# AllenNeuralDynamics/aind-smartspim-destripe

Measured on AMD Instinct MI355X. Metric: 2048x2048 uint16 slices/s destriped, higher is better.
Workload: dtype f32

## Files before the change

### aind_smartspim_destripe_amd/csrc/dsx.hip

```cpp
#include <hip/hip_runtime.h>
#include <dlfcn.h>
#include <math.h>
#include <rccl/rccl.h>
#include <stdio.h>
#include <stdlib.h>
#include <string.h>

#include <string>
#include <vector>

#include "../../include/dsx.h"
#include "dsx_kernels.h"
#include "dsx_retile.h"
#include "dsx_pyramid.h"
#include "dsx_wavelet.h"
#include "dsx_plan.h"
#include "dsx_io.h"
#include "dsx_streaks.h"
#include "dsx_zenc_kernels.h"
#include "dsx_zdec_kernels.h"

namespace {

thread_local std::string g_init_error;
// ... 3 lines not shown
                                     "k_rowfilter",       "k_inv_march(pyramid)", "k_inv_march(final)"};

struct ProfRec {
  int cls;
  hipEvent_t e0, e1;
};

}

struct DsxTuning {
  int row_wpb = 0;
  int march_waves = 256 * 16;
  bool no_quant = false;
  int seg_min_rows = 4;
  bool no_fuse = false;
  bool no_fuse_inv = false;
  bool no_pair = false;
  int hist_rows = 0;
  int fwd_wpb = 8, inv_wpb = 8;
  bool no_row_multi = false;
  int row_multi_alone = 48;
  int helper = -1;
  bool no_pipeline = false;
#ifdef DSX_DIAG
  int skip_hist = 0, skip_row = 0, skip_from = 1000;
#endif
};

struct dsx_ctx {
  int device = 0;
  DsxTuning tune;
  hipStream_t stream_ = nullptr;
  std::string err;
  bool planned = false;
  dsx::Plan plan;
  dsx::HostCfg cfg[2];
  double high_int = 2700.0;
  int max_batch = 0;
  float fg_cutoff = 383.12503f;
  float* d_ws = nullptr;
  char* d_ctl = nullptr;
  size_t ctl_zero_bytes = 0;
  dsx::PlaneStats* d_stats = nullptr;
  unsigned* d_minmax = nullptr;
  unsigned* d_hist = nullptr;
  float* d_thr = nullptr;
  float* d_otsu = nullptr;
  int* d_cfg = nullptr;
  double* d_means = nullptr;
  dsx::C32* d_consts = nullptr;
  size_t consts_bytes = 0;
  float* d_flat = nullptr;
  float* d_dark = nullptr;
  bool own_shading = false;
  int dark_h = 0, dark_w = 0;
  void* d_stage_in = nullptr;
  void* d_stage_out = nullptr;
  size_t stage_in_bytes = 0, stage_out_bytes = 0;
  int last_n = 0;
  int stop_after = 0;
  hipEvent_t t0 = nullptr, t1 = nullptr;
  bool profiling = false;
  std::vector<ProfRec> prof;
  size_t workspace_bytes = 0;
  int wl_len = 0;
  int wl_bank_len = 0;
  bool wl_set = false;
  float wl[4][dsx::kMaxTaps] = {};
  float wl_bank[4][dsx::kMaxTaps] = {};
  unsigned* h_sticky = nullptr;
  uint8_t* zenc_slots = nullptr;
  uint32_t* zenc_sizes = nullptr;
  size_t zenc_blocks = 0;
  uint8_t* zenc_lits = nullptr;
  size_t zenc_lit_blocks = 0;
  uint8_t* zdec_scratch = nullptr;
  size_t zdec_bytes = 0;
  unsigned* d_sticky = nullptr;
  bool stack_mode = false;
  bool no_fuse_rf = false;
  bool fuse_rf_wide = false;
  int ablate = 0;
// ... 65 lines not shown
}

int env_int(const char* name, int fallback) {
  const char* v = getenv(name);
  return (v && *v) ? atoi(v) : fallback;
}

void read_tuning(DsxTuning& t) {
  t.row_wpb = env_int("DSX_ROW_WPB", 0);
  if (t.row_wpb != 0) t.row_wpb = std::max(4, std::min(t.row_wpb, (int)dsx::kRowMaxWaves));
  t.march_waves = std::max(64, env_int("DSX_MARCH_WAVES", 256 * 16));
  t.no_quant = env_int("DSX_NO_QUANT", 0) != 0;
  t.seg_min_rows = std::max(2, env_int("DSX_SEG_MIN_ROWS", 4));
  t.no_fuse = env_int("DSX_NO_FUSE", 0) != 0;
  t.no_fuse_inv = env_int("DSX_NO_FUSE_INV", 0) != 0;
  t.no_pair = env_int("DSX_NO_PAIR", 0) != 0;
  t.hist_rows = std::max(0, env_int("DSX_HIST_ROWS", 0));
  t.fwd_wpb = env_int("DSX_FWD_WPB", 8) == 4 ? 4 : 8;
  t.inv_wpb = env_int("DSX_INV_WPB", 8) == 4 ? 4 : 8;
  t.no_row_multi = env_int("DSX_NO_ROW_MULTI", 0) != 0;
  t.row_multi_alone = std::max(0, env_int("DSX_ROW_MULTI_ALONE", 48));
  t.helper = getenv("DSX_HELPER") ? (env_int("DSX_HELPER", 0) != 0 ? 1 : 0) : -1;
  t.no_pipeline = env_int("DSX_NO_PIPELINE", 0) != 0;
#ifdef DSX_DIAG
  t.skip_hist = env_int("DSX_SKIP_HIST", 0);
  t.skip_row = env_int("DSX_SKIP_ROW", 0);
  t.skip_from = env_int("DSX_SKIP_COARSE", 1000);
#endif
}

int fail(dsx_ctx* c, int code, const std::string& msg) {
  if (c) c->err = msg;
  else g_init_error = msg;
  return code;
}

hipStream_t use_main(dsx_ctx* c) {
  for (int i = 1; i < c->joins_pending; ++i) (void)hipStreamWaitEvent(c->stream_, c->ev_join[i], 0);
  c->joins_pending = 0;
  ++c->main_ops;
  return c->stream_;
}

#define DSX_HIP(call)                                                                    \
  do {                                                                                   \
    hipError_t e_ = (call);                                                              \
// ... 3 lines not shown

void drop_graphs(dsx_ctx* c) {
  for (auto& g : c->graphs)
    if (g.exec) (void)hipGraphExecDestroy(g.exec);
  c->graphs.clear();
}

void free_plan_buffers(dsx_ctx* c) {
  drop_graphs(c);
  auto fr = [](void* p) { if (p) (void)hipFree(p); };
  fr(c->d_ws); c->d_ws = nullptr;
  fr(c->d_ctl); c->d_ctl = nullptr;
  fr(c->d_thr); c->d_thr = nullptr;
  fr(c->d_otsu); c->d_otsu = nullptr;
  fr(c->d_cfg); c->d_cfg = nullptr;
  fr(c->d_means); c->d_means = nullptr;
  fr(c->d_consts); c->d_consts = nullptr;
  if (c->own_shading) { fr(c->d_flat); fr(c->d_dark); }
  c->d_flat = c->d_dark = nullptr;
  c->own_shading = false;
  fr(c->d_stage_in); c->d_stage_in = nullptr; c->stage_in_bytes = 0;
  fr(c->d_stage_out); c->d_stage_out = nullptr; c->stage_out_bytes = 0;
  c->planned = false;
}

struct LaunchScope {
  dsx_ctx* c;
  bool on;
  ProfRec r;
  LaunchScope(dsx_ctx* c_, int cls) : c(c_), on(c_->profiling) {
    if (on) {
      r.cls = cls;
      (void)hipEventCreate(&r.e0);
      (void)hipEventCreate(&r.e1);
      (void)hipEventRecord(r.e0, c->stream_);
    }
  }
  ~LaunchScope() {
    if (on) {
      (void)hipEventRecord(r.e1, c->stream_);
      c->prof.push_back(r);
    }
  }
};

int rowfilter_waves_per_block(int M) {
// ... 23 lines not shown
  const int wpb = force_wpb ? force_wpb : ((CPL > 18 || a_in.M >= 1024) ? 4 : rowfilter_waves_per_block(a_in.M));
  const size_t smem = (size_t)a_in.M * (wpb + 1) * sizeof(float2);
  const dsx::RowArgs& a = a_in;
  const dim3 grid((npairs + wpb - 1) / wpb, nb);
  hipLaunchKernelGGL((dsx::k_rowfilter<CPL, GF, NT, HALO, PLAN>), grid, dim3(64 * wpb), smem, s, a);
  return hipGetLastError();
}

hipError_t launch_rowfilter_wide(const dsx::RowArgs& a, int npairs, int nb, hipStream_t s) {
  static bool attr_set[64] = {};
  int dev = 0;
  (void)hipGetDevice(&dev);
  if (!attr_set[dev & 63]) {
    hipError_t e = hipFuncSetAttribute((const void*)dsx::k_rowfilter_wide, hipFuncAttributeMaxDynamicSharedMemorySize,
                                       (int)(dsx::kWideMaxLen * sizeof(float2)));
    if (e != hipSuccess) return e;
    attr_set[dev & 63] = true;
  }
  if (a.M > dsx::kWideMaxLen || a.w >= 65536) return hipErrorInvalidValue;
  hipLaunchKernelGGL(dsx::k_rowfilter_wide, dim3(npairs, nb), dim3(dsx::kWideThreads), (size_t)a.M * sizeof(float2), s, a);
  return hipGetLastError();
}

hipError_t dispatch_rowfilter(const dsx::RowArgs& a, int npairs, int nb, hipStream_t s) {
  const int cpl = (a.M + 63) / 64;
  if (cpl > 36) return launch_rowfilter_wide(a, npairs, nb, s);
  const int gf = a.w >> 8, nt = (a.w - (gf << 8) + 63) >> 6;
  auto plan_is = [&](int m, int r0, int r1, int r2) {
    return a.M == m && a.npass == 3 && a.radix[0] == r0 && a.radix[1] == r1 && a.radix[2] == r2;
  };
  if (cpl <= 2) return launch_rowfilter<2>(a, npairs, nb, s);
  if (cpl <= 4) return launch_rowfilter<4>(a, npairs, nb, s);
  if (cpl <= 6) return launch_rowfilter<6>(a, npairs, nb, s);
  if (cpl <= 10) return launch_rowfilter<10>(a, npairs, nb, s);
  if (cpl <= 18) {
    if (gf == 4 && nt == 1 && a.K == 0) {
      if (plan_is(1026, 19, 9, 6))
        return launch_rowfilter<18, 4, 1, 0, 1>(a, npairs, nb, s);
      return launch_rowfilter<18, 4, 1, 0>(a, npairs, nb, s);
    }
    if (gf == 2 && nt == 1 && a.K > 0) {
      if (plan_is(1071, 17, 9, 7))
        return launch_rowfilter<18, 2, 1, 1, 2>(a, npairs, nb, s);
      return launch_rowfilter<18, 2, 1, 1>(a, npairs, nb, s);
    }
    if (gf == 1 && nt == 4 && a.K > 0) {
      if (plan_is(1024, 16, 8, 8)) return launch_rowfilter<18, 1, 4, 1, 5>(a, npairs, nb, s);
      if (plan_is(960, 15, 8, 8)) return launch_rowfilter<18, 1, 4, 1, 6>(a, npairs, nb, s);
    }
// ... 28 lines not shown
  if (!attr_set[dev & 63]) {
    hipError_t e = hipFuncSetAttribute((const void*)kern, hipFuncAttributeMaxDynamicSharedMemorySize, 160 * 1024);
    if (e != hipSuccess) return e;
    attr_set[dev & 63] = true;
  }
  const size_t smem = (size_t)a.r.M * (dsx::kRfWaves + 1) * sizeof(float2);
  const int np = (a.f.hout + 1) / 2;
  int nblk = (np + dsx::kRfRows - 1) / dsx::kRfRows;
#if DSX_RF_XCD
  nblk = (nblk + 7) / 8 * 8;
#endif
  const dim3 grid(nblk, nb);
  hipLaunchKernelGGL(kern, grid, dim3(64 * dsx::kRfWaves), smem, s, a);
  return hipGetLastError();
}

hipError_t launch_rowfinal(int plan, const dsx::RowFinalArgs& a, int nb, hipStream_t s) {
  if (plan == 1) return launch_rowfinal_t<18, 4, 1, 0, 1>(a, nb, s);
  if (plan == 3) return launch_rowfinal_t<36, 3, 4, 1, 3>(a, nb, s);
  if (plan == 4) return launch_rowfinal_t<36, 3, 3, 1, 4>(a, nb, s);
  return hipErrorInvalidValue;
}

hipError_t launch_rowfilter_multi(const dsx::RowMultiArgs& a_in, const int* npairs, int nb, hipStream_t s) {
  static bool attr_set[64] = {};
  int dev = 0;
  (void)hipGetDevice(&dev);
  if (!attr_set[dev & 63]) {
    hipError_t e = hipFuncSetAttribute((const void*)dsx::k_rowfilter_multi<6>, hipFuncAttributeMaxDynamicSharedMemorySize, 160 * 1024);
    if (e != hipSuccess) return e;
    attr_set[dev & 63] = true;
  }
  const int wpb = dsx::kRowMaxWaves;
  dsx::RowMultiArgs a = a_in;
  int blocks = 0, max_m = 1;
  for (int i = 0; i < a.nlev; ++i) {
    blocks += (npairs[i] + wpb - 1) / wpb;
    a.blk_end[i] = blocks;
    max_m = std::max(max_m, a.lv[i].M);
  }
  const size_t smem = (size_t)max_m * (wpb + 1) * sizeof(float2);
  hipLaunchKernelGGL(dsx::k_rowfilter_multi<6>, dim3(blocks, nb), dim3(64 * wpb), smem, s, a);
  return hipGetLastError();
}

void march_segments(int nb, int nstrips, int rows, int* nseg, int* rows_per_seg, int wpb = 0, int halo_rows = 0,
                    bool coarse = false) {
  const int target_waves = tune().march_waves;
  const bool no_quant = tune().no_quant;
  int want = (target_waves + nb * nstrips - 1) / (nb * nstrips);
  const int seg_min_coarse = tune().seg_min_rows;
  const int seg_min_rows = coarse ? seg_min_coarse : 24;
  const int max_seg = std::max(1, rows / seg_min_rows);
  want = std::max(1, std::min(want, max_seg));
  if (wpb > 0 && !no_quant) {
    static int cus = 0;
    if (cus == 0) {
      int dev = 0;
      hipDeviceProp_t prop;
      if (hipGetDevice(&dev) == hipSuccess && hipGetDeviceProperties(&prop, dev) == hipSuccess) cus = prop.multiProcessorCount;
      if (cus <= 0) cus = 256;
    }
    const long long slots = (long long)cus * (16 / wpb);
    double best = 1e300;
    int best_n = want;
// ... 188 lines not shown
    a.sticky = ctx->d_sticky;
    a.shared = ctx->stack_mode ? 1 : 0;
    LaunchScope ls(ctx, KC_OTSU);
    hipLaunchKernelGGL(dsx::k_otsu, dim3(L, nb), dim3(64), 0, s, a);
    DSX_HIP(hipGetLastError());
    if (d_cfg_used)
      DSX_HIP(hipMemcpyAsync(d_cfg_used, v.cfg, sizeof(int32_t) * nb, hipMemcpyDeviceToDevice, s));
  } else if (d_cfg_used) {
    DSX_HIP(hipMemsetAsync(d_cfg_used, 0, sizeof(int32_t) * nb, s));
  }
  if (ctx->stop_after == 1) return DSX_OK;

  const bool split_inv = split && fuse21;
  if (split_inv) {
    DSX_HIP(hipEventRecord(v.ev[2], s));
    DSX_HIP(hipStreamWaitEvent(v.helper, v.ev[2], 0));
  }
  dsx::RowArgs row1;
  memset(&row1, 0, sizeof(row1));
  const bool no_multi = ctx->tune.no_row_multi;
  dsx::RowMultiArgs multi;
  memset(&multi, 0, sizeof(multi));
  int multi_pairs[dsx::kRowMultiMax] = {};
  for (int l = 0; l < L && l < skip_from; ++l) {
    hipStream_t rs = (split_inv && l < 2) ? v.helper : s;
    if ((skip_row >> l) & 1) continue;
    const dsx::LevelPlan& lp = p.lv[l];
    dsx::RowArgs a;
    memset(&a, 0, sizeof(a));
    a.ws = v.ws;
    a.ws_plane_stride = p.plane_floats;
    a.da_off = lp.da_off;
    a.h = lp.h; a.w = lp.w; a.ld = lp.ld;
    a.thr = v.thr;
    a.cfg = v.cfg;
    a.lvl = l; a.L = L;
    a.lvl_active[0] = p.cfg_levels[0];
    a.lvl_active[1] = p.cfg_levels[1];
    a.M = lp.M; a.K = lp.K;
    a.npass = lp.npass;
    for (int i = 0; i < lp.npass; ++i) a.radix[i] = lp.radix[i];
    a.tw = (const float2*)(ctx->d_consts + lp.tw_off);
    a.g[0] = (const float2*)(ctx->d_consts + lp.g_off[0]);
    a.g[1] = (const float2*)(ctx->d_consts + lp.g_off[1]);
    a.kcut[0] = lp.kcut[0];
    a.kcut[1] = lp.kcut[1];
    a.inv_M = 1.0f / (float)lp.M;
    a.ablate = ctx->ablate;
    if (fuse_rf && l == 0) {
      row1 = a;
      continue;
    }
    const int npairs = (lp.h + 1) / 2;
    const int multi_alone = ctx->tune.row_multi_alone;
    if (!no_multi && (!v.alone || nb <= multi_alone) && rs == s && a.M <= 6 * 64 && multi.nlev < dsx::kRowMultiMax) {
      multi_pairs[multi.nlev] = npairs;
      multi.lv[multi.nlev++] = a;
      continue;
    }
    LaunchScope ls(ctx, KC_ROW);
    DSX_HIP(dispatch_rowfilter(a, npairs, nb, rs));
  }
  if (multi.nlev == 1) {
    LaunchScope ls(ctx, KC_ROW);
    DSX_HIP(dispatch_rowfilter(multi.lv[0], multi_pairs[0], nb, s));
  } else if (multi.nlev > 1) {
    LaunchScope ls(ctx, KC_ROW);
    DSX_HIP(launch_rowfilter_multi(multi, multi_pairs, nb, s));
  }
  if (split_inv) DSX_HIP(hipEventRecord(v.ev[3], v.helper));
  if (ctx->stop_after == 2) return DSX_OK;

  for (int l = L - 1; l >= (L > 0 ? 0 : -1); --l) {
    if (fuse21 && l == 1) continue;
    if (l >= skip_from) continue;
    if (generic) {
      dsx::GenInvArgs g;
      memset(&g, 0, sizeof(g));
      const dsx::LevelPlan& lp = p.lv[l];
      g.ws = v.ws;
      g.ws_plane_stride = p.plane_floats;
      g.c_off = lp.aa_off; g.d_off = lp.da_off;
      g.hc = lp.h; g.wc = lp.w; g.ldc = lp.lda; g.ldd = lp.ld;
      g.has_c = (l < L - 1) ? 1 : 0;
      g.has_pyr = 1;
      g.F = ctx->wl_len;
      memcpy(g.lo, ctx->wl[2], sizeof(float) * ctx->wl_len);
      memcpy(g.hi, ctx->wl[3], sizeof(float) * ctx->wl_len);
      const bool last_g = (l == 0);
      if (!last_g) {
        const dsx::LevelPlan& lo = p.lv[l - 1];
// ... 1432 lines not shown
  DSX_HIP(hipStreamSynchronize(use_main(ctx)));
  if (int rc = check_sticky(ctx)) return rc;
  double m[2];
  int c = 0;
  DSX_HIP(hipMemcpy(m, ctx->d_means + 2 * plane, sizeof(m), hipMemcpyDeviceToHost));
  DSX_HIP(hipMemcpy(&c, ctx->d_cfg + plane, sizeof(int), hipMemcpyDeviceToHost));
  if (fore_mean) *fore_mean = m[0];
  if (back_mean) *back_mean = m[1];
  if (cfg_used) *cfg_used = c;
  return DSX_OK;
}
int dsx_get_thresholds(dsx_ctx* ctx, int plane, int level, float* otsu, float* threshold) {
  if (!ctx) return DSX_EINVAL;
  if (!ctx->planned) return fail(ctx, DSX_ENOPLAN, "dsx_plan has not been called");
  if (plane < 0 || plane >= ctx->last_n || level < 0 || level >= ctx->plan.L)
    return fail(ctx, DSX_EINVAL, "plane / level index out of range");
  DSX_HIP(hipSetDevice(ctx->device));
  DSX_HIP(hipStreamSynchronize(use_main(ctx)));
  const size_t i = (size_t)plane * ctx->plan.L + level;
  if (otsu) DSX_HIP(hipMemcpy(otsu, ctx->d_otsu + i, sizeof(float), hipMemcpyDeviceToHost));
  if (threshold) DSX_HIP(hipMemcpy(threshold, ctx->d_thr + i, sizeof(float), hipMemcpyDeviceToHost));
  return DSX_OK;
}
int dsx_get_level(dsx_ctx* ctx, int plane, int level, int stage, float* out) {
  if (!ctx || !out) return DSX_EINVAL;
  if (!ctx->planned) return fail(ctx, DSX_ENOPLAN, "dsx_plan has not been called");
  if (plane < 0 || plane >= ctx->last_n || level < 0 || level >= ctx->plan.L)
    return fail(ctx, DSX_EINVAL, "plane / level index out of range");
  DSX_HIP(hipSetDevice(ctx->device));
  DSX_HIP(hipStreamSynchronize(use_main(ctx)));
  const dsx::LevelPlan& lp = ctx->plan.lv[level];
  const long long off = (stage == DSX_STAGE_APPROX) ? lp.aa_off : lp.da_off;
  const int pitch = (stage == DSX_STAGE_APPROX) ? lp.lda : lp.ld;
  const float* src = ctx->d_ws + (size_t)plane * ctx->plan.plane_floats + off;
  DSX_HIP(hipMemcpy2D(out, sizeof(float) * lp.w, src, sizeof(float) * pitch, sizeof(float) * lp.w, lp.h,
                      hipMemcpyDeviceToHost));
  return DSX_OK;
}

int dsx_plan_streaks(dsx_ctx* ctx, int height, int width, int max_batch, const dsx_streaks_cfg* cfg) {
  if (!ctx) return DSX_EINVAL;
  if (!cfg) return fail(ctx, DSX_EINVAL, "config is NULL");
  if (height < 1 || width < 1) return fail(ctx, DSX_EINVAL, "plane must be at least 1 x 1");
  if (max_batch < 1) return fail(ctx, DSX_EINVAL, "max_batch must be >= 1");
  if (!(cfg->sigma_fg > 0.f) || !(cfg->sigma_bg > 0.f)) return fail(ctx, DSX_EINVAL, "sigma must be positive");
  if (!(cfg->crossover > 0.f)) return fail(ctx, DSX_EINVAL, "crossover must be positive");
// ... 81 lines not shown
```

### aind_smartspim_destripe_amd/csrc/dsx_kernels.h

```cpp
#ifndef DSX_KERNELS_H
#define DSX_KERNELS_H

#include <type_traits>
#include <hip/hip_runtime.h>
#include <stdint.h>

#include "dsx_fft_core.h"

#ifndef DSX_NT
#define DSX_NT 1
#endif
#ifndef DSX_MEDIAN_BALLOT
#define DSX_MEDIAN_BALLOT 1
#endif
#ifndef DSX_FWD_STEADY
#define DSX_FWD_STEADY 1
#endif
#ifndef DSX_RF_XCD
#define DSX_RF_XCD 0
#endif
#ifndef DSX_INV_MINW
#define DSX_INV_MINW 1
#endif
#ifndef DSX_FWD_PRUNE
#define DSX_FWD_PRUNE 1
#endif
#ifndef DSX_SWZ
#define DSX_SWZ 1
#endif
#ifndef DSX_FWD_MINW
// ... 1053 lines not shown
    const double t = fmin(otsu >= 0 ? sqrt(otsu) : 0.0, (double)a.max_thr[cfg]);
    a.otsu[pl] = (float)otsu;
    a.thr[pl] = (float)t;
  }
}

struct RowArgs {
  float* ws;
  long long ws_plane_stride;
  long long da_off;
  int h, w, ld;
  const float* thr;
  const int* cfg;
  int lvl, L;
  int lvl_active[2];
  int M, K;
  int npass;
  int radix[kMaxPasses];
  const float2* tw;
  const float2* g[2];
  int kcut[2];
  float inv_M;
  int ablate;
};

__device__ __forceinline__ unsigned f32_key(float v) {
  const unsigned b = as_u32(v);
  return (b & 0x80000000u) ? ~b : (b | 0x80000000u);
}
__device__ __forceinline__ float key_f32(unsigned k) {
  return as_f32((k & 0x80000000u) ? (k & 0x7FFFFFFFu) : ~k);
}

template <int R, int CPL, int JK = (R - 1) / 2, int KO = (R - 1) / 2, class IX = dsx_idx_plain>
__device__ __forceinline__ void fft_pass(float2* buf, const float2* tw, int M, int s, float inv_s,
                                         int lane) {
  constexpr int MAXB = (CPL + R - 1) / R;
  const int nb = M / R;
  const bool unit_tw = (s * R == M);
  dsx_c32 v[MAXB][R];
#pragma unroll
  for (int i = 0; i < MAXB; ++i) {
    const int b = lane + kWave * i;
    if (b < nb) dsx_bfly_load<R, JK, IX>((const dsx_c32*)buf, b, nb, v[i]);
  }
  wave_sync();
// ... 143 lines not shown
    const int jk = (kcut + 53) / 54;
    if (jk <= 2) run_first_pruned<CPL, 2>(buf, tw, lane);
    else if (jk <= 4) run_first_pruned<CPL, 4>(buf, tw, lane);
    else run<CPL>(buf, tw, lane);
  }
};
template <>
struct StaticFft<2> {
  static constexpr int M = 1071;
  static constexpr bool kSwz = false;
  static constexpr int kRadix[3] = {17, 9, 7};
  template <int CPL>
  static __device__ __forceinline__ void run(float2* buf, const float2* tw, int lane) {
    fft_static_passes<CPL, 1071, 1, 17, 9, 7>(buf, tw, lane);
  }
  template <int CPL>
  static __device__ __forceinline__ void run_forward(float2* buf, const float2* tw, int lane, int) { run<CPL>(buf, tw, lane); }
  template <int CPL>
  static __device__ __forceinline__ void run_inverse(float2* buf, const float2* tw, int lane, int) {
    run<CPL>(buf, tw, lane);
  }
};

#define DSX_STATIC_FFT(ID, LEN, R0, R1, R2, SWZ)                                                   \
  template <>                                                                                      \
  struct StaticFft<ID> {                                                                           \
    static constexpr int M = LEN;                                                                  \
    static constexpr bool kSwz = SWZ;                                                              \
    template <int CPL>                                                                             \
    static __device__ __forceinline__ void run(float2* buf, const float2* tw, int lane) {          \
      if constexpr (SWZ) fft_static_passes_swz<CPL, LEN, 1, R0, R1, R2>(buf, tw, lane);            \
      else fft_static_passes<CPL, LEN, 1, R0, R1, R2>(buf, tw, lane);                              \
    }                                                                                              \
    template <int CPL>                                                                             \
    static __device__ __forceinline__ void run_forward(float2* buf, const float2* tw, int lane, int) { \
      run<CPL>(buf, tw, lane);                                                                     \
    }                                                                                              \
    template <int CPL>                                                                             \
    static __device__ __forceinline__ void run_inverse(float2* buf, const float2* tw, int lane, int) { \
      run<CPL>(buf, tw, lane);                                                                     \
    }                                                                                              \
  };
DSX_STATIC_FFT(3, 2048, 16, 16, 8, DSX_SWZ != 0)
DSX_STATIC_FFT(4, 1815, 15, 11, 11, false)
DSX_STATIC_FFT(5, 1024, 16, 8, 8, DSX_SWZ != 0)
DSX_STATIC_FFT(6, 960, 15, 8, 8, false)
#undef DSX_STATIC_FFT

typedef short dsx_s16x2 __attribute__((ext_vector_type(2)));

__device__ __forceinline__ dsx_s16x2 as_s16x2(unsigned u) {
  union { unsigned u; dsx_s16x2 v; } c;
  c.u = u;
  return c.v;
}
__device__ __forceinline__ unsigned as_u32(dsx_s16x2 v) {
  union { unsigned u; dsx_s16x2 v; } c;
  c.v = v;
  return c.u;
}

template <int CPL>
struct RowSlots {
  static constexpr int GV = CPL / 4;
  static constexpr int E = 4 * GV + 4;
};
template <int E>
struct SlotMask { typedef unsigned long long type; };
template <> struct SlotMask<4> { typedef unsigned type; };
template <> struct SlotMask<8> { typedef unsigned type; };
// ... 371 lines not shown
  const int tid = threadIdx.x, lane = tid & 63, wave = tid >> 6;
  const int M = (PLAN_ > 0) ? StaticFft<PLAN_>::M : a.M;
  rf_pair_body<CPL, GF_, NT_, HALO_, PLAN_, false>(a, dsx_smem, dsx_smem + (long long)M * (1 + wave), tid, blockDim.x, lane,
                                                   blockIdx.x * (blockDim.x >> 6) + wave, blockIdx.y);
}

constexpr int kRowMultiMax = 8;
struct RowMultiArgs {
  int nlev;
  int blk_end[kRowMultiMax];
  RowArgs lv[kRowMultiMax];
};

template <int CPL>
__global__ __launch_bounds__(64 * kRowMaxWaves, row_waves_per_simd<CPL>()) void k_rowfilter_multi(RowMultiArgs args) {
  extern __shared__ __attribute__((aligned(16))) float2 dsx_smem[];
  const int tid = threadIdx.x, lane = tid & 63, wave = tid >> 6;
  int ent = 0;
  while (ent + 1 < args.nlev && (int)blockIdx.x >= args.blk_end[ent]) ++ent;
  const RowArgs& a = args.lv[ent];
  const int bx = (int)blockIdx.x - (ent > 0 ? args.blk_end[ent - 1] : 0);
  rf_pair_body<CPL, -1, -1, -1, 0, false>(a, dsx_smem, dsx_smem + (long long)a.M * (1 + wave), tid, blockDim.x, lane,
                                          bx * (blockDim.x >> 6) + wave, blockIdx.y);
}

constexpr int kWideThreads = 512;
constexpr int kWideCpl = 36;
constexpr int kWideMaxLen = kWideThreads * kWideCpl;

__device__ __forceinline__ unsigned wide_block_sum(unsigned v, unsigned* s_red, int& turn) {
  v = __reduce_add_sync(~0ull, v);
  unsigned* slot = s_red + ((turn & 1) ? (kWideThreads / 64) : 0);
  if ((threadIdx.x & 63) == 0) slot[threadIdx.x >> 6] = v;
  __syncthreads();
  unsigned t = 0;
#pragma unroll
  for (int w = 0; w < kWideThreads / 64; ++w) t += slot[w];
  ++turn;
  return t;
}
__device__ __forceinline__ unsigned wide_block_min(unsigned v, unsigned* s_red, int& turn) {
  v = __reduce_min_sync(~0ull, v);
  unsigned* slot = s_red + ((turn & 1) ? (kWideThreads / 64) : 0);
  if ((threadIdx.x & 63) == 0) slot[threadIdx.x >> 6] = v;
  __syncthreads();
  unsigned t = ~0u;
// ... 889 lines not shown
```

### aind_smartspim_destripe_amd/csrc/dsx_plan.h

```cpp
#ifndef DSX_PLAN_H
#define DSX_PLAN_H

#include <math.h>
#include <stdint.h>
#include <stdlib.h>

#include <algorithm>
#include <string>
#include <vector>

namespace dsx {

constexpr int kPlanMaxLevels = 16;
constexpr int kPlanMaxPasses = 16;
constexpr int kFilterLen = 6;
constexpr int kMaxFftLen = 64 * 36;
constexpr int kMaxWideLen = 512 * 36;

struct HostCfg {
  int level;
  double sigma;
  double max_threshold;
};

// ... 13 lines not shown
  long long g_off[2];
  int kcut[2];
};

struct Plan {
  int H = 0, W = 0, Hout = 0, Wout = 0;
  int L = 0;
  int cfg_levels[2] = {0, 0};
  LevelPlan lv[kPlanMaxLevels];
  long long plane_floats = 0;
  std::vector<C32> consts;
};

inline int dwt_max_level(int n, int filter_len = kFilterLen) {
  if (filter_len < 2 || n < filter_len - 1) return 0;
  int l = (int)floor(log2((double)(n / (filter_len - 1))));
  return l < 0 ? 0 : l;
}

inline int cpl_class(int m) {
  const int cpl = (m + 63) / 64;
  for (int c : {2, 4, 6, 10, 18, 36}) if (cpl <= c) return c;
  return 1 << 30;
}

constexpr int kRegRadix[] = {2, 3, 4, 5, 6, 7, 8, 9, 10, 11, 12, 13, 15, 16, 17, 19, 20, 25};
inline double round_cost(int r) {
  switch (r) {
    case 2: return 28;
    case 3: return 37;
    case 4: return 64;
    case 5: return 84;
    case 6: return 82;
    case 7: return 109;
    case 8: return 133;
    case 9: return 151;
    case 10: return 214;
    case 11: return 191;
    case 12: return 251;
    case 13: return 238;
    case 15: return 352;
    case 16: return 337;
    case 17: return 359;
    case 19: return 408;
    case 20: return 520;
    case 25: return 708;
// ... 208 lines not shown
```

### aind_smartspim_destripe_amd/engine.py

```python

import ctypes
import os

import numpy as np

from . import wavelets

_HERE = os.path.dirname(os.path.abspath(__file__))
LIB_PATH = os.environ.get("DSX_LIB") or os.path.join(_HERE, "_lib", "libdsx_hip.so")

DSX_U16, DSX_F32 = 0, 1
DSX_WAVELET_DB3 = 3
DSX_WAVELET_BANK = 0
STAGE_APPROX, STAGE_DETAIL = 0, 1
STREAM_COMPUTE, STREAM_UPLOAD, STREAM_DOWNLOAD = 0, 1, 2

TASK_FILL, TASK_COPY, TASK_STORED, TASK_ZSTD, TASK_LZ4 = 0, 1, 2, 3, 4
TASK_SHUFFLE, TASK_SPLIT, TASK_BITSHUFFLE = 0x100, 0x200, 0x400
ZDEC_ZSTD, ZDEC_ANY = 0, 1
ROUTE_DEVICE, ROUTE_HOST, ROUTE_FILL = 0, 1, 2
TASK_DTYPE = np.dtype([("src", "<u8"), ("dst", "<u8"), ("src_len", "<u4"), ("dst_len", "<u4"), ("kind", "<u4"),
                       ("chunk", "<u4")])

COMM_ID_BYTES = 128
_ERRORS = {-1: "DSX_EINVAL", -2: "DSX_ENOPLAN", -3: "DSX_EHIP", -4: "DSX_ENOMEM", -5: "DSX_ELIMIT",
           -6: "DSX_ECOMM", -7: "DSX_EIO", -8: "DSX_EVALUE"}

EXPORTED_SYMBOLS = [
    "dsx_init", "dsx_destroy", "dsx_last_error", "dsx_device_count", "dsx_plan", "dsx_plan_info", "dsx_set_wavelet", "dsx_graph_stats",
    "dsx_set_shading_device", "dsx_constants_device", "dsx_run_host", "dsx_run_device", "dsx_sync",
    "dsx_malloc", "dsx_free", "dsx_memcpy_h2d", "dsx_memcpy_d2h", "dsx_memcpy_d2d",
    "dsx_timer_start", "dsx_timer_stop", "dsx_profile_enable", "dsx_profile_read",
    "dsx_get_stats", "dsx_get_thresholds", "dsx_get_level", "dsx_set_stop_after", "dsx_set_stack_mode",
    "dsx_bricks_to_planes_u16", "dsx_planes_to_bricks_u16", "dsx_downsample2_u16",
    "dsx_flatfield_correction", "dsx_flatfield_correction_rows", "dsx_foreground_background",
    "dsx_comm_unique_id", "dsx_comm_init", "dsx_comm_destroy", "dsx_comm_broadcast", "dsx_comm_allreduce_f64",
    "dsx_malloc_host", "dsx_free_host", "dsx_memcpy_h2d_async", "dsx_memcpy_d2h_async",
    "dsx_stream_wait", "dsx_stream_sync", "dsx_event_record", "dsx_event_sync",
    "dsx_io_read_chunks", "dsx_io_write_chunks", "dsx_io_write_chunks_blosc", "dsx_blosc_decode", "dsx_blosc_encode",
    "dsx_png_unfilter", "dsx_plan_streaks", "dsx_get_streaks_threshold",
    "dsx_blosc_encode_device", "dsx_blosc_encode_ref", "dsx_blosc_encode_device_ex", "dsx_blosc_encode_ref_ex",
    "dsx_io_read_frames", "dsx_io_read_frames_ex", "dsx_blosc_decode_device", "dsx_blosc_decode_ref",
    "dsx_pyramid_work_bytes", "dsx_pyramid_block_u16", "dsx_pyramid_block_ref",
    "dsx_pyramid_bricks_u16", "dsx_pyramid_bricks_ref",
]


def frame_tasks_per_chunk(chunk_bytes):
    return int(chunk_bytes) // 8192 + 1


def decode_task(src, dst, src_len, dst_len, kind, chunk=0):
    t = np.zeros(1, TASK_DTYPE)
    t[0] = (src, dst, src_len, dst_len, kind, chunk)
    return t

# ... 72 lines not shown
    lib.dsx_plan.argtypes = [vp, i32, i32, i32, ctypes.POINTER(_Cfg), ctypes.POINTER(_Cfg),
                             ctypes.c_double, vp, vp, i32, i32]
    lib.dsx_plan_info.argtypes = [vp, ctypes.POINTER(_PlanInfo)]
    lib.dsx_set_shading_device.argtypes = [vp, vp, vp, i32, i32]
    lib.dsx_constants_device.argtypes = [vp, ctypes.POINTER(vp), ctypes.POINTER(ctypes.c_size_t)]
    lib.dsx_run_host.argtypes = [vp, vp, i32, i32, vp, i32, vp]
    lib.dsx_run_device.argtypes = [vp, vp, i32, i32, vp, i32, vp]
    lib.dsx_sync.argtypes = [vp]
    lib.dsx_malloc.argtypes = [vp, ctypes.c_size_t, ctypes.POINTER(vp)]
    lib.dsx_free.argtypes = [vp, vp]
    lib.dsx_memcpy_h2d.argtypes = [vp, vp, vp, ctypes.c_size_t]
    lib.dsx_memcpy_d2h.argtypes = [vp, vp, vp, ctypes.c_size_t]
    lib.dsx_memcpy_d2d.argtypes = [vp, vp, vp, ctypes.c_size_t]
    lib.dsx_timer_start.argtypes = [vp]
    lib.dsx_timer_stop.argtypes = [vp, f32p]
    lib.dsx_profile_enable.argtypes = [vp, i32]
    lib.dsx_profile_read.argtypes = [vp, i32, f32p, ctypes.POINTER(ctypes.c_int32),
                                     ctypes.POINTER(ctypes.c_char_p), ctypes.POINTER(i32)]
    lib.dsx_get_stats.argtypes = [vp, i32, ctypes.POINTER(ctypes.c_double),
                                  ctypes.POINTER(ctypes.c_double), ctypes.POINTER(ctypes.c_int32)]
    lib.dsx_get_thresholds.argtypes = [vp, i32, i32, f32p, f32p]
    lib.dsx_get_level.argtypes = [vp, i32, i32, i32, vp]
    lib.dsx_set_stop_after.argtypes = [vp, i32]
    lib.dsx_set_stack_mode.argtypes = [vp, i32]
    lib.dsx_graph_stats.argtypes = [vp, ctypes.POINTER(ctypes.c_uint64), ctypes.POINTER(ctypes.c_uint64)]
    lib.dsx_set_wavelet.argtypes = [vp] + [ctypes.POINTER(ctypes.c_double)] * 4 + [i32]
    lib.dsx_bricks_to_planes_u16.argtypes = [vp, vp, vp] + [i32] * 7
    lib.dsx_planes_to_bricks_u16.argtypes = [vp, vp, vp] + [i32] * 7
    lib.dsx_downsample2_u16.argtypes = [vp, vp, vp, i32, i32, i32]
    lib.dsx_foreground_background.argtypes = [vp, vp, i32, ctypes.c_size_t, ctypes.c_float,
                                              ctypes.POINTER(ctypes.c_double), ctypes.POINTER(ctypes.c_double), vp]
    lib.dsx_flatfield_correction.argtypes = [vp, vp, i32, i32, i32, vp, vp, i32, i32, ctypes.c_float, vp]
    lib.dsx_flatfield_correction_rows.argtypes = [vp, vp, i32, i32, i32, vp, vp, i32, i32, ctypes.c_float, vp, vp]
    lib.dsx_comm_unique_id.argtypes = [vp, ctypes.c_char_p, ctypes.c_size_t]
    lib.dsx_comm_init.argtypes = [vp, ctypes.c_char_p, ctypes.c_size_t, i32, i32]
    lib.dsx_comm_destroy.argtypes = [vp]
    lib.dsx_comm_broadcast.argtypes = [vp, vp, ctypes.c_size_t, i32]
    lib.dsx_comm_allreduce_f64.argtypes = [vp, ctypes.POINTER(ctypes.c_double), i32, i32]
    lib.dsx_malloc_host.argtypes = [vp, ctypes.c_size_t, ctypes.POINTER(vp)]
    lib.dsx_free_host.argtypes = [vp, vp]
    lib.dsx_memcpy_h2d_async.argtypes = [vp, vp, vp, ctypes.c_size_t, i32]
    lib.dsx_memcpy_d2h_async.argtypes = [vp, vp, vp, ctypes.c_size_t, i32]
    lib.dsx_stream_wait.argtypes = [vp, i32, i32]
    lib.dsx_stream_sync.argtypes = [vp, i32]
    lib.dsx_event_record.argtypes = [vp, i32, i32]
    lib.dsx_event_sync.argtypes = [vp, i32]
# ... 469 lines not shown
                raise ValueError(self._lib.dsx_last_error(self._ctx).decode())
            self._check(rc)
            return bufs[3].download((H, W), np.uint16)
        finally:
            for b in bufs:
                b.free()

    def set_stack_mode(self, on):
        self._check(self._lib.dsx_set_stack_mode(self._ctx, 1 if on else 0))

    def set_stop_after(self, stage):
        self._check(self._lib.dsx_set_stop_after(self._ctx, int(stage)))

    def stats(self, plane):
        f, b, c = ctypes.c_double(), ctypes.c_double(), ctypes.c_int32()
        self._check(self._lib.dsx_get_stats(self._ctx, int(plane), ctypes.byref(f), ctypes.byref(b), ctypes.byref(c)))
        return f.value, b.value, c.value

    def thresholds(self, plane, level):
        o, t = ctypes.c_float(), ctypes.c_float()
        self._check(self._lib.dsx_get_thresholds(self._ctx, int(plane), int(level), ctypes.byref(o), ctypes.byref(t)))
        return o.value, t.value

    def level_array(self, plane, level, stage=STAGE_DETAIL):
        out = np.empty(self.level_shape(level), dtype=np.float32)
        self._check(self._lib.dsx_get_level(self._ctx, int(plane), int(level), int(stage),
                                            out.ctypes.data_as(ctypes.c_void_p)))
        return out


def _pyramid_table(zyx, chunks, z0s, zero, rows):
    n = len(chunks)
    table = (_PyramidLevel * max(n, 1))()
    for i, ck in enumerate(chunks):
        z0 = int(z0s[i]) if z0s is not None else 0
        share = int(zyx[0]) >> (i + 1)
        need = max(1, -(-(z0 + share) // int(ck[0])))
        table[i] = _PyramidLevel(int(ck[0]), int(ck[1]), int(ck[2]), int(rows[i]) if rows is not None else need, z0,
                                 1 if zero is None or zero[i] else 0)
    return table


def pyramid_level_elems(zyx, level, chunk, rows=1):
    nby = -(-(int(zyx[1]) >> level) // int(chunk[1]))
    nbx = -(-(int(zyx[2]) >> level) // int(chunk[2]))
    return int(rows) * nby * nbx * int(chunk[0]) * int(chunk[1]) * int(chunk[2])
# ... 144 lines not shown
```

### include/dsx.h

```cpp
#ifndef DSX_H
#define DSX_H

#include <stddef.h>
#include <stdint.h>

#ifdef __cplusplus
extern "C" {
#endif

#define DSX_VERSION 100

#define DSX_OK 0
#define DSX_EINVAL (-1)
#define DSX_ENOPLAN (-2)
#define DSX_EHIP (-3)
#define DSX_ENOMEM (-4)
#define DSX_ELIMIT (-5)
#define DSX_ECOMM (-6)
#define DSX_EIO (-7)
#define DSX_EVALUE (-8)

#define DSX_U16 0
#define DSX_F32 1

// ... 144 lines not shown
#define DSX_COMM_ID_BYTES 128
int dsx_comm_unique_id(dsx_ctx* ctx, char* id, size_t id_bytes);
int dsx_comm_init(dsx_ctx* ctx, const char* id, size_t id_bytes, int rank, int world);
int dsx_comm_destroy(dsx_ctx* ctx);
int dsx_comm_broadcast(dsx_ctx* ctx, void* d_buf, size_t bytes, int root);
int dsx_comm_allreduce_f64(dsx_ctx* ctx, double* values, int n, int op);

typedef struct dsx_streaks_cfg {
  int32_t wavelet;
  int32_t level;
  float sigma_fg;
  float sigma_bg;
  float crossover;
  int32_t otsu;
  float threshold;
} dsx_streaks_cfg;
int dsx_plan_streaks(dsx_ctx* ctx, int height, int width, int max_batch, const dsx_streaks_cfg* cfg);
int dsx_get_streaks_threshold(dsx_ctx* ctx, int plane, float* threshold);

int dsx_get_stats(dsx_ctx* ctx, int plane, double* fore_mean, double* back_mean,
                  int32_t* cfg_used);
int dsx_get_thresholds(dsx_ctx* ctx, int plane, int level, float* otsu, float* threshold);
int dsx_get_level(dsx_ctx* ctx, int plane, int level, int stage, float* out);
int dsx_set_stop_after(dsx_ctx* ctx, int stage);

#ifdef __cplusplus
}
#endif
#endif
```

Before: 71380.

## Specialise coarse-level row filters with compile-time static FFT plans

Adds static FFT definitions for the small coarse-level transform sizes (260, 132, 144, 36, 20, 12) and a table that matches plan levels to them. Both the single-level dispatch and the multi-level fused row filter kernel then launch template-specialised bodies with fixed radices, CPL, group and halo parameters, in place of the generic runtime-plan path. This is meant to cut runtime indexing, branching and register overhead in the many small coarse-level FFTs. The cost is larger code and more template instantiations. The specialisation only applies when every level matches the table, otherwise it falls back to the generic kernels.

```diff
diff --git a/aind_smartspim_destripe_amd/csrc/dsx.hip b/aind_smartspim_destripe_amd/csrc/dsx.hip
--- a/aind_smartspim_destripe_amd/csrc/dsx.hip
+++ b/aind_smartspim_destripe_amd/csrc/dsx.hip
@@ -49,6 +49,7 @@
   int row_multi_alone = 48;
   int helper = -1;
   bool no_pipeline = false;
+  bool rf_coarse_static = true;
 #ifdef DSX_DIAG
   int skip_hist = 0, skip_row = 0, skip_from = 1000;
 #endif
@@ -85,6 +86,7 @@
   void* d_stage_out = nullptr;
   size_t stage_in_bytes = 0, stage_out_bytes = 0;
   int last_n = 0;
+  int rf_ran[dsx::kPlanMaxLevels] = {};
   int stop_after = 0;
   hipEvent_t t0 = nullptr, t1 = nullptr;
   bool profiling = false;
@@ -196,6 +198,7 @@
   t.row_multi_alone = std::max(0, env_int("DSX_ROW_MULTI_ALONE", 48));
   t.helper = getenv("DSX_HELPER") ? (env_int("DSX_HELPER", 0) != 0 ? 1 : 0) : -1;
   t.no_pipeline = env_int("DSX_NO_PIPELINE", 0) != 0;
+  t.rf_coarse_static = env_int("DSX_RF_COARSE_STATIC", 1) != 0;
 #ifdef DSX_DIAG
   t.skip_hist = env_int("DSX_SKIP_HIST", 0);
   t.skip_row = env_int("DSX_SKIP_ROW", 0);
@@ -245,6 +248,7 @@
   fr(c->d_stage_in); c->d_stage_in = nullptr; c->stage_in_bytes = 0;
   fr(c->d_stage_out); c->d_stage_out = nullptr; c->stage_out_bytes = 0;
   c->planned = false;
+  memset(c->rf_ran, 0, sizeof(c->rf_ran));
 }
 
 struct LaunchScope {
@@ -314,9 +318,38 @@
   return hipGetLastError();
 }
 
-hipError_t dispatch_rowfilter(const dsx::RowArgs& a, int npairs, int nb, hipStream_t s) {
+void coarse_static_rows(const dsx::Plan& p, const DsxTuning& t, int* rows) {
+  bool all = t.rf_coarse_static;
+  for (int l = 0; l < p.L; ++l) {
+    const dsx::LevelPlan& lp = p.lv[l];
+    rows[l] = (lp.M <= 6 * 64) ? dsx::coarse_static_index(lp.w, lp.M, lp.K, lp.npass, lp.radix) : -1;
+    all = all && (lp.M > 6 * 64 || rows[l] >= 0);
+  }
+  if (!all)
+    for (int l = 0; l < p.L; ++l) rows[l] = -1;
+}
+
+template <int I>
+hipError_t launch_rowfilter_coarse(const dsx::RowArgs& a, int npairs, int nb, hipStream_t s) {
+  typedef dsx::RfCoarseBody<I> B;
+  return launch_rowfilter<B::kCpl, B::kGf, B::kNt, B::kHalo, B::kPlan>(a, npairs, nb, s);
+}
+
+hipError_t dispatch_rowfilter(const dsx::RowArgs& a, int npairs, int nb, hipStream_t s, int* ran) {
   const int cpl = (a.M + 63) / 64;
+  ran[a.lvl] = 0;
   if (cpl > 36) return launch_rowfilter_wide(a, npairs, nb, s);
+  static_assert(dsx::kCoarseStaticCount == 6, "one case per row of kCoarseStatic");
+  if (a.body > 0 && a.body <= dsx::kCoarseStaticCount) ran[a.lvl] = dsx::kCoarseStatic[a.body - 1].id;
+  switch (a.body) {
+    case 1: return launch_rowfilter_coarse<0>(a, npairs, nb, s);
+    case 2: return launch_rowfilter_coarse<1>(a, npairs, nb, s);
+    case 3: return launch_rowfilter_coarse<2>(a, npairs, nb, s);
+    case 4: return launch_rowfilter_coarse<3>(a, npairs, nb, s);
+    case 5: return launch_rowfilter_coarse<4>(a, npairs, nb, s);
+    case 6: return launch_rowfilter_coarse<5>(a, npairs, nb, s);
+    default: break;
+  }
   const int gf = a.w >> 8, nt = (a.w - (gf << 8) + 63) >> 6;
   auto plan_is = [&](int m, int r0, int r1, int r2) {
     return a.M == m && a.npass == 3 && a.radix[0] == r0 && a.radix[1] == r1 && a.radix[2] == r2;
@@ -391,25 +424,32 @@
   return hipErrorInvalidValue;
 }
 
-hipError_t launch_rowfilter_multi(const dsx::RowMultiArgs& a_in, const int* npairs, int nb, hipStream_t s) {
+hipError_t launch_rowfilter_multi(const dsx::RowMultiArgs& a_in, const int* npairs, int nb, hipStream_t s, int* ran) {
+  const auto k_static = dsx::k_rowfilter_multi_static<dsx::RfCoarseBody<0>, dsx::RfCoarseBody<1>, dsx::RfCoarseBody<2>,
+                                                      dsx::RfCoarseBody<3>, dsx::RfCoarseBody<4>, dsx::RfCoarseBody<5>>;
   static bool attr_set[64] = {};
   int dev = 0;
   (void)hipGetDevice(&dev);
   if (!attr_set[dev & 63]) {
     hipError_t e = hipFuncSetAttribute((const void*)dsx::k_rowfilter_multi<6>, hipFuncAttributeMaxDynamicSharedMemorySize, 160 * 1024);
+    if (e == hipSuccess) e = hipFuncSetAttribute((const void*)k_static, hipFuncAttributeMaxDynamicSharedMemorySize, 160 * 1024);
     if (e != hipSuccess) return e;
     attr_set[dev & 63] = true;
   }
   const int wpb = dsx::kRowMaxWaves;
   dsx::RowMultiArgs a = a_in;
   int blocks = 0, max_m = 1;
+  bool all_static = true;
   for (int i = 0; i < a.nlev; ++i) {
     blocks += (npairs[i] + wpb - 1) / wpb;
     a.blk_end[i] = blocks;
     max_m = std::max(max_m, a.lv[i].M);
-  }
+    all_static = all_static && a.lv[i].body > 0 && a.lv[i].body <= dsx::kCoarseStaticCount;
+  }
+  for (int i = 0; i < a.nlev; ++i) ran[a.lv[i].lvl] = all_static ? dsx::kCoarseStatic[a.lv[i].body - 1].id : 0;
   const size_t smem = (size_t)max_m * (wpb + 1) * sizeof(float2);
-  hipLaunchKernelGGL(dsx::k_rowfilter_multi<6>, dim3(blocks, nb), dim3(64 * wpb), smem, s, a);
+  if (all_static) hipLaunchKernelGGL(k_static, dim3(blocks, nb), dim3(64 * wpb), smem, s, a);
+  else hipLaunchKernelGGL(dsx::k_rowfilter_multi<6>, dim3(blocks, nb), dim3(64 * wpb), smem, s, a);
   return hipGetLastError();
 }
 
@@ -644,6 +684,8 @@
   dsx::RowMultiArgs multi;
   memset(&multi, 0, sizeof(multi));
   int multi_pairs[dsx::kRowMultiMax] = {};
+  int body_rows[dsx::kPlanMaxLevels];
+  coarse_static_rows(p, ctx->tune, body_rows);
   for (int l = 0; l < L && l < skip_from; ++l) {
     hipStream_t rs = (split_inv && l < 2) ? v.helper : s;
     if ((skip_row >> l) & 1) continue;
@@ -669,6 +711,7 @@
     a.kcut[1] = lp.kcut[1];
     a.inv_M = 1.0f / (float)lp.M;
     a.ablate = ctx->ablate;
+    a.body = body_rows[l] + 1;
     if (fuse_rf && l == 0) {
       row1 = a;
       continue;
@@ -681,14 +724,14 @@
       continue;
     }
     LaunchScope ls(ctx, KC_ROW);
-    DSX_HIP(dispatch_rowfilter(a, npairs, nb, rs));
+    DSX_HIP(dispatch_rowfilter(a, npairs, nb, rs, ctx->rf_ran));
   }
   if (multi.nlev == 1) {
     LaunchScope ls(ctx, KC_ROW);
-    DSX_HIP(dispatch_rowfilter(multi.lv[0], multi_pairs[0], nb, s));
+    DSX_HIP(dispatch_rowfilter(multi.lv[0], multi_pairs[0], nb, s, ctx->rf_ran));
   } else if (multi.nlev > 1) {
     LaunchScope ls(ctx, KC_ROW);
-    DSX_HIP(launch_rowfilter_multi(multi, multi_pairs, nb, s));
+    DSX_HIP(launch_rowfilter_multi(multi, multi_pairs, nb, s, ctx->rf_ran));
   }
   if (split_inv) DSX_HIP(hipEventRecord(v.ev[3], v.helper));
   if (ctx->stop_after == 2) return DSX_OK;
@@ -2167,6 +2210,10 @@
   if (threshold) DSX_HIP(hipMemcpy(threshold, ctx->d_thr + i, sizeof(float), hipMemcpyDeviceToHost));
   return DSX_OK;
 }
+int dsx_rowfilter_body(const dsx_ctx* ctx, int level) {
+  if (!ctx || !ctx->planned || ctx->streaks || level < 0 || level >= ctx->plan.L) return -1;
+  return ctx->rf_ran[level];
+}
 int dsx_get_level(dsx_ctx* ctx, int plane, int level, int stage, float* out) {
   if (!ctx || !out) return DSX_EINVAL;
   if (!ctx->planned) return fail(ctx, DSX_ENOPLAN, "dsx_plan has not been called");
diff --git a/aind_smartspim_destripe_amd/csrc/dsx_kernels.h b/aind_smartspim_destripe_amd/csrc/dsx_kernels.h
--- a/aind_smartspim_destripe_amd/csrc/dsx_kernels.h
+++ b/aind_smartspim_destripe_amd/csrc/dsx_kernels.h
@@ -6,6 +6,7 @@
 #include <stdint.h>
 
 #include "dsx_fft_core.h"
+#include "dsx_plan.h"
 
 #ifndef DSX_NT
 #define DSX_NT 1
@@ -1105,6 +1106,7 @@
   int kcut[2];
   float inv_M;
   int ablate;
+  int body;
 };
 
 __device__ __forceinline__ unsigned f32_key(float v) {
@@ -1294,15 +1296,19 @@
   }
 };
 
-#define DSX_STATIC_FFT(ID, LEN, R0, R1, R2, SWZ)                                                   \
+template <int... R>
+constexpr int dsx_pack_count() { return (int)sizeof...(R); }
+#define DSX_STATIC_FFT(ID, LEN, SWZ, ...)                                                          \
   template <>                                                                                      \
   struct StaticFft<ID> {                                                                           \
     static constexpr int M = LEN;                                                                  \
     static constexpr bool kSwz = SWZ;                                                              \
+    static constexpr int kRadix[3] = {__VA_ARGS__};                                                \
+    static constexpr int kPasses = dsx_pack_count<__VA_ARGS__>();                                  \
     template <int CPL>                                                                             \
     static __device__ __forceinline__ void run(float2* buf, const float2* tw, int lane) {          \
-      if constexpr (SWZ) fft_static_passes_swz<CPL, LEN, 1, R0, R1, R2>(buf, tw, lane);            \
-      else fft_static_passes<CPL, LEN, 1, R0, R1, R2>(buf, tw, lane);                              \
+      if constexpr (SWZ) fft_static_passes_swz<CPL, LEN, 1, __VA_ARGS__>(buf, tw, lane);           \
+      else fft_static_passes<CPL, LEN, 1, __VA_ARGS__>(buf, tw, lane);                             \
     }                                                                                              \
     template <int CPL>                                                                             \
     static __device__ __forceinline__ void run_forward(float2* buf, const float2* tw, int lane, int) { \
@@ -1313,11 +1319,29 @@
       run<CPL>(buf, tw, lane);                                                                     \
     }                                                                                              \
   };
-DSX_STATIC_FFT(3, 2048, 16, 16, 8, DSX_SWZ != 0)
-DSX_STATIC_FFT(4, 1815, 15, 11, 11, false)
-DSX_STATIC_FFT(5, 1024, 16, 8, 8, DSX_SWZ != 0)
-DSX_STATIC_FFT(6, 960, 15, 8, 8, false)
+DSX_STATIC_FFT(3, 2048, DSX_SWZ != 0, 16, 16, 8)
+DSX_STATIC_FFT(4, 1815, false, 15, 11, 11)
+DSX_STATIC_FFT(5, 1024, DSX_SWZ != 0, 16, 8, 8)
+DSX_STATIC_FFT(6, 960, false, 15, 8, 8)
+DSX_STATIC_FFT(7, 260, false, 13, 5, 4)
+DSX_STATIC_FFT(8, 132, false, 11, 3, 4)
+DSX_STATIC_FFT(9, 144, false, 6, 6, 4)
+DSX_STATIC_FFT(10, 36, false, 6, 6)
+DSX_STATIC_FFT(11, 20, false, 5, 4)
+DSX_STATIC_FFT(12, 12, false, 3, 4)
 #undef DSX_STATIC_FFT
+
+template <int ID>
+constexpr bool coarse_static_matches() {
+  const CoarseStaticPlan* e = coarse_static_by_id(ID);
+  if (!e || e->M != StaticFft<ID>::M || e->npass != StaticFft<ID>::kPasses) return false;
+  for (int i = 0; i < e->npass; ++i)
+    if (e->radix[i] != StaticFft<ID>::kRadix[i]) return false;
+  return true;
+}
+static_assert(coarse_static_matches<7>() && coarse_static_matches<8>() && coarse_static_matches<9>() &&
+                  coarse_static_matches<10>() && coarse_static_matches<11>() && coarse_static_matches<12>(),
+              "StaticFft<7 ... 12> and dsx_plan.h: kCoarseStatic disagree");
 
 typedef short dsx_s16x2 __attribute__((ext_vector_type(2)));
 
@@ -1735,6 +1759,51 @@
   const int bx = (int)blockIdx.x - (ent > 0 ? args.blk_end[ent - 1] : 0);
   rf_pair_body<CPL, -1, -1, -1, 0, false>(a, dsx_smem, dsx_smem + (long long)a.M * (1 + wave), tid, blockDim.x, lane,
                                           bx * (blockDim.x >> 6) + wave, blockIdx.y);
+}
+
+template <int CPL_, int GF_, int NT_, int HALO_, int PLAN_>
+struct RfBody {
+  static constexpr int kCpl = CPL_, kGf = GF_, kNt = NT_, kHalo = HALO_, kPlan = PLAN_;
+};
+template <int I>
+using RfCoarseBody = RfBody<kCoarseStatic[I].cpl, kCoarseStatic[I].gf, kCoarseStatic[I].nt, (kCoarseStatic[I].K > 0) ? 1 : 0,
+                            kCoarseStatic[I].id>;
+template <int I, class B0, class... REST>
+struct rf_body_at { typedef typename rf_body_at<I - 1, REST...>::type type; };
+template <class B0, class... REST>
+struct rf_body_at<0, B0, REST...> { typedef B0 type; };
+
+template <int I, class... BODY>
+__device__ __forceinline__ void rf_static_body(const RowArgs& a, float2* smem, int tid, int nthreads, int lane, int wave,
+                                               int bx, int plane) {
+  if constexpr (I < (int)sizeof...(BODY)) {
+    typedef typename rf_body_at<I, BODY...>::type B;
+    constexpr int M = StaticFft<B::kPlan>::M;
+    static_assert(M > 0 && M <= 64 * B::kCpl, "the body's CPL class must hold its transform");
+    rf_pair_body<B::kCpl, B::kGf, B::kNt, B::kHalo, B::kPlan, false>(a, smem, smem + (long long)M * (1 + wave), tid, nthreads,
+                                                                    lane, bx * (nthreads >> 6) + wave, plane);
+  }
+}
+
+template <class... BODY>
+__global__ __launch_bounds__(64 * kRowMaxWaves, row_waves_per_simd<6>()) void k_rowfilter_multi_static(RowMultiArgs args) {
+  static_assert(sizeof...(BODY) == 6, "the switch below has one case per body");
+  extern __shared__ __attribute__((aligned(16))) float2 dsx_smem[];
+  const int tid = threadIdx.x, lane = tid & 63, wave = tid >> 6;
+  int ent = 0;
+  while (ent + 1 < args.nlev && (int)blockIdx.x >= args.blk_end[ent]) ++ent;
+  const RowArgs& a = args.lv[ent];
+  const int bx = (int)blockIdx.x - (ent > 0 ? args.blk_end[ent - 1] : 0);
+  const int nthreads = blockDim.x, plane = blockIdx.y;
+  switch (a.body) {
+    case 1: rf_static_body<0, BODY...>(a, dsx_smem, tid, nthreads, lane, wave, bx, plane); break;
+    case 2: rf_static_body<1, BODY...>(a, dsx_smem, tid, nthreads, lane, wave, bx, plane); break;
+    case 3: rf_static_body<2, BODY...>(a, dsx_smem, tid, nthreads, lane, wave, bx, plane); break;
+    case 4: rf_static_body<3, BODY...>(a, dsx_smem, tid, nthreads, lane, wave, bx, plane); break;
+    case 5: rf_static_body<4, BODY...>(a, dsx_smem, tid, nthreads, lane, wave, bx, plane); break;
+    case 6: rf_static_body<5, BODY...>(a, dsx_smem, tid, nthreads, lane, wave, bx, plane); break;
+    default: break;
+  }
 }
 
 constexpr int kWideThreads = 512;
diff --git a/aind_smartspim_destripe_amd/csrc/dsx_plan.h b/aind_smartspim_destripe_amd/csrc/dsx_plan.h
--- a/aind_smartspim_destripe_amd/csrc/dsx_plan.h
+++ b/aind_smartspim_destripe_amd/csrc/dsx_plan.h
@@ -59,6 +59,34 @@
   const int cpl = (m + 63) / 64;
   for (int c : {2, 4, 6, 10, 18, 36}) if (cpl <= c) return c;
   return 1 << 30;
+}
+
+struct CoarseStaticPlan {
+  int id, w, M, K, npass, radix[3], cpl, gf, nt;
+};
+constexpr CoarseStaticPlan kCoarseStatic[] = {
+    {7, 260, 260, 0, 3, {13, 5, 4}, 6, 1, 1},
+    {8, 132, 132, 0, 3, {11, 3, 4}, 4, 0, 3},
+    {9, 68, 144, 34, 3, {6, 6, 4}, 4, 0, 2},
+    {10, 36, 36, 0, 2, {6, 6, 0}, 2, 0, 1},
+    {11, 20, 20, 0, 2, {5, 4, 0}, 2, 0, 1},
+    {12, 12, 12, 0, 2, {3, 4, 0}, 2, 0, 1},
+};
+constexpr int kCoarseStaticCount = (int)(sizeof(kCoarseStatic) / sizeof(kCoarseStatic[0]));
+constexpr const CoarseStaticPlan* coarse_static_by_id(int id) {
+  for (int i = 0; i < kCoarseStaticCount; ++i)
+    if (kCoarseStatic[i].id == id) return &kCoarseStatic[i];
+  return nullptr;
+}
+inline int coarse_static_index(int w, int M, int K, int npass, const int* radix) {
+  for (int i = 0; i < kCoarseStaticCount; ++i) {
+    const CoarseStaticPlan& e = kCoarseStatic[i];
+    if (e.w != w || e.M != M || e.K != K || e.npass != npass) continue;
+    bool same = true;
+    for (int j = 0; j < npass; ++j) same = same && (e.radix[j] == radix[j]);
+    if (same) return i;
+  }
+  return -1;
 }
 
 constexpr int kRegRadix[] = {2, 3, 4, 5, 6, 7, 8, 9, 10, 11, 12, 13, 15, 16, 17, 19, 20, 25};
diff --git a/aind_smartspim_destripe_amd/engine.py b/aind_smartspim_destripe_amd/engine.py
--- a/aind_smartspim_destripe_amd/engine.py
+++ b/aind_smartspim_destripe_amd/engine.py
@@ -32,6 +32,7 @@
     "dsx_malloc", "dsx_free", "dsx_memcpy_h2d", "dsx_memcpy_d2h", "dsx_memcpy_d2d",
     "dsx_timer_start", "dsx_timer_stop", "dsx_profile_enable", "dsx_profile_read",
     "dsx_get_stats", "dsx_get_thresholds", "dsx_get_level", "dsx_set_stop_after", "dsx_set_stack_mode",
+    "dsx_rowfilter_body",
     "dsx_bricks_to_planes_u16", "dsx_planes_to_bricks_u16", "dsx_downsample2_u16",
     "dsx_flatfield_correction", "dsx_flatfield_correction_rows", "dsx_foreground_background",
     "dsx_comm_unique_id", "dsx_comm_init", "dsx_comm_destroy", "dsx_comm_broadcast", "dsx_comm_allreduce_f64",
@@ -150,6 +151,7 @@
     lib.dsx_get_thresholds.argtypes = [vp, i32, i32, f32p, f32p]
     lib.dsx_get_level.argtypes = [vp, i32, i32, i32, vp]
     lib.dsx_set_stop_after.argtypes = [vp, i32]
+    lib.dsx_rowfilter_body.argtypes = [vp, i32]
     lib.dsx_set_stack_mode.argtypes = [vp, i32]
     lib.dsx_graph_stats.argtypes = [vp, ctypes.POINTER(ctypes.c_uint64), ctypes.POINTER(ctypes.c_uint64)]
     lib.dsx_set_wavelet.argtypes = [vp] + [ctypes.POINTER(ctypes.c_double)] * 4 + [i32]
@@ -665,6 +667,12 @@
         self._check(self._lib.dsx_get_thresholds(self._ctx, int(plane), int(level), ctypes.byref(o), ctypes.byref(t)))
         return o.value, t.value
 
+    def rowfilter_body(self, level):
+        r = int(self._lib.dsx_rowfilter_body(self._ctx, int(level)))
+        if r < 0:
+            raise ValueError("rowfilter_body: no plan, or no level {}".format(level))
+        return r
+
     def level_array(self, plane, level, stage=STAGE_DETAIL):
         out = np.empty(self.level_shape(level), dtype=np.float32)
         self._check(self._lib.dsx_get_level(self._ctx, int(plane), int(level), int(stage),
diff --git a/include/dsx.h b/include/dsx.h
--- a/include/dsx.h
+++ b/include/dsx.h
@@ -190,6 +190,7 @@
                   int32_t* cfg_used);
 int dsx_get_thresholds(dsx_ctx* ctx, int plane, int level, float* otsu, float* threshold);
 int dsx_get_level(dsx_ctx* ctx, int plane, int level, int stage, float* out);
+int dsx_rowfilter_body(const dsx_ctx* ctx, int level);
 int dsx_set_stop_after(dsx_ctx* ctx, int stage);
 
 #ifdef __cplusplus
```

After: 72980 (median of 6 runs). 1.02x the previous value.
